# UVA-Computer-Vision-Lab/midvision-probe

Hardware: AMD Instinct MI355X
Metric: images/sec feature-extract+probe-step, ViT-B/16 224^2 (higher is better)
Workload: dtype f16x2 (compensated fp16 pairs of activations and frozen weights, two f16 MFMA products per contraction, fp32 accumulate, feature error as bf16x3; attention: Q.K^T the same two products over compensated pairs, P.V fp16 probabilities x (fp16 + bf16) V; probe, fp32 residual/LN/softmax/loss as in bf16x3

## Files before the change

### midvision-probe_amd/csrc/attention.hip

```cpp
#include "mvp_common.h"

#ifndef MVP_ATT_NT
#define MVP_ATT_NT 0
#endif
#ifndef MVP_ATT_LD_AUX
#define MVP_ATT_LD_AUX 0
#endif
namespace {

#ifndef MVP_ATT_PRIO
#define MVP_ATT_PRIO 0
#endif
#ifndef MVP_ATT_STAGGER
#define MVP_ATT_STAGGER 0
#endif
#if MVP_ATT_PRIO
#define ATT_PRIO(v) __builtin_amdgcn_s_setprio(v)
#else
#define ATT_PRIO(v)
#endif
#ifndef MVP_ATT_ABLATE
#define MVP_ATT_ABLATE 0
#endif
constexpr int TILE = 64 * 128;
constexpr float ATT_DEFER = 6.0f;

template <int SPLIT>
struct AttnState {
  bf16x8_t q_hi[2][2], q_lo[2][2];
  f32x4_t o_acc[4][2];
  float m_run[2], l_run[2];
};

struct AttnBias {
  const float* row[2];
  float scale;
  const float* rel;
  unsigned qoff[2];
  int Kh, Kw, q16, r16;
};

template <int SPLIT, bool LAST, int VF16 = 0, int BIAS = 0>
__device__ __forceinline__ void attn_tile(AttnState<SPLIT>& st, const char* kb, const char* vb, int key0, int N, float cs, int lane,
                                          const AttnBias& ab = AttnBias{}) {
  static_assert(!VF16 || SPLIT == 3, "the fp16-probability form belongs to the bf16x3 mode");
  const int g = lane >> 4, c16 = lane & 15;
  const int nsub = LAST ? min(4, (N - key0 + 15) >> 4) : 4;
  f32x4_t s[4][2];
#pragma unroll
  for (int t = 0; t < 4; ++t)
#pragma unroll
    for (int qt = 0; qt < 2; ++qt) s[t][qt] = f32x4_t{0.f, 0.f, 0.f, 0.f};
  f32x4_t bv[4][2];
  if constexpr (BIAS == 1) {
#pragma unroll
    for (int t = 0; t < 4; ++t)
#pragma unroll
      for (int qt = 0; qt < 2; ++qt)
        bv[t][qt] = (LAST && t >= nsub) ? f32x4_t{0.f, 0.f, 0.f, 0.f} : *(const f32x4_t*)(ab.row[qt] + key0 + t * 16);
  }
  ATT_PRIO(1);
#pragma unroll
  for (int ks = 0; ks < (MVP_ATT_ABLATE == 3 ? 0 : 2); ++ks) {
    const int coff = (((ks << 2) + g) ^ (lane & 7)) << 4;
#pragma unroll
    for (int t = 0; t < 4; ++t) {
      if (LAST && t >= nsub) continue;
      const char* ka = kb + (t * 16 + c16) * 128 + coff;
      const bf16x8_t k_hi = *(const bf16x8_t*)ka;
      if (VF16 == 2) {
        const f16x8_t k_lo = *(const f16x8_t*)(ka + TILE);
        const f16x8_t k_h = __builtin_bit_cast(f16x8_t, k_hi);
#pragma unroll
        for (int qt = 0; qt < 2; ++qt) {
          s[t][qt] = __builtin_amdgcn_mfma_f32_16x16x32_f16(k_lo, __builtin_bit_cast(f16x8_t, st.q_lo[qt][ks]), s[t][qt], 0, 0, 0);
          s[t][qt] = __builtin_amdgcn_mfma_f32_16x16x32_f16(k_h, __builtin_bit_cast(f16x8_t, st.q_hi[qt][ks]), s[t][qt], 0, 0, 0);
        }
        continue;
      }
      if (SPLIT == 3) {
        const bf16x8_t k_lo = *(const bf16x8_t*)(ka + TILE);
#pragma unroll
        for (int qt = 0; qt < 2; ++qt) {
          s[t][qt] = __builtin_amdgcn_mfma_f32_16x16x32_bf16(k_lo, st.q_hi[qt][ks], s[t][qt], 0, 0, 0);
          s[t][qt] = __builtin_amdgcn_mfma_f32_16x16x32_bf16(k_hi, st.q_lo[qt][ks], s[t][qt], 0, 0, 0);
        }
      }
#pragma unroll
      for (int qt = 0; qt < 2; ++qt)
        s[t][qt] = __builtin_amdgcn_mfma_f32_16x16x32_bf16(k_hi, st.q_hi[qt][ks], s[t][qt], 0, 0, 0);
    }
  }
  ATT_PRIO(0);
  if constexpr (BIAS == 1) {
#pragma unroll
    for (int t = 0; t < 4; ++t)
#pragma unroll
      for (int qt = 0; qt < 2; ++qt)
#pragma unroll
        for (int j = 0; j < 4; ++j) s[t][qt][j] = __builtin_fmaf(s[t][qt][j], ab.scale, bv[t][qt][j]);
  }
  if constexpr (BIAS == 2) {
    unsigned k0 = (unsigned)(key0 + g * 4);
    asm volatile("" : "+v"(k0));
    const unsigned Kw4 = (unsigned)ab.Kw << 2, Kh4 = (unsigned)ab.Kh << 2;
    const unsigned q0y = k0 / (unsigned)ab.Kw;
    unsigned ty = q0y << 2, tx = (k0 - q0y * (unsigned)ab.Kw) << 2;
    const char* base = (const char*)ab.rel;
#pragma unroll
    for (int t = 0; t < 4; ++t) {
      if (!(LAST && t >= nsub)) {
        unsigned ky = ty, kx = tx;
#pragma unroll
        for (int j = 0; j < 4; ++j) {
          const bool dead = LAST && (int)k0 + t * 16 + j >= N;
          const unsigned yy = dead ? 0u : ky, xx = (dead ? 0u : kx) + Kh4;
#pragma unroll
          for (int qt = 0; qt < 2; ++qt)
            s[t][qt][j] = __builtin_fmaf(s[t][qt][j], ab.scale, *(const float*)(base + (ab.qoff[qt] + yy)) + *(const float*)(base + (ab.qoff[qt] + xx)));
          kx += 4;
          if (kx == Kw4) {
            kx = 0;
            ky += 4;
          }
        }
      }
      ty += ab.q16;
      tx += ab.r16;
      if (tx >= Kw4) {
        tx -= Kw4;
        ty += 4;
      }
      __builtin_amdgcn_sched_barrier(0);
    }
  }
  const int kbase = key0 + g * 4;
  bf16x8_t p_hi[2][2], p_lo[2][2];
  f16x8_t p_h[2][2];
#pragma unroll
  for (int qt = 0; qt < 2; ++qt) {
    if (VF16 && MVP_ATT_ABLATE != 1) {
      float tmax = -1e30f;
#pragma unroll
      for (int t = 0; t < 4; ++t)
#pragma unroll
        for (int j = 0; j < 4; ++j) {
          if (LAST) s[t][qt][j] = ((kbase + t * 16 + j) < N) ? s[t][qt][j] : -1e30f;
          tmax = fmaxf(tmax, s[t][qt][j]);
        }
      tmax = fmaxf(tmax, __shfl_xor(tmax, 16, 64));
      tmax = fmaxf(tmax, __shfl_xor(tmax, 32, 64));
      if (__builtin_amdgcn_ballot_w64((tmax - st.m_run[qt]) * cs > ATT_DEFER) != 0) {
        const float m_new = fmaxf(st.m_run[qt], tmax);
        const float alpha = __builtin_amdgcn_exp2f((st.m_run[qt] - m_new) * cs);
        st.m_run[qt] = m_new;
        st.l_run[qt] *= alpha;
#pragma unroll
        for (int dt = 0; dt < 4; ++dt) st.o_acc[dt][qt] *= alpha;
      }
      const float mc = st.m_run[qt] * cs;
      float psum = 0.f;
#pragma unroll
      for (int t = 0; t < 4; ++t)
#pragma unroll
        for (int j = 0; j < 4; ++j) {
          const float pv = (LAST && t >= nsub) ? 0.f : __builtin_amdgcn_exp2f(s[t][qt][j] * cs - mc);
          psum += pv;
          p_h[qt][t >> 1][(t & 1) * 4 + j] = (_Float16)pv;
          p_lo[qt][t >> 1][(t & 1) * 4 + j] = (__bf16)pv;
        }
      st.l_run[qt] += psum;
      continue;
    }
    if (MVP_ATT_ABLATE == 1) {
#pragma unroll
      for (int t = 0; t < 4; ++t)
#pragma unroll
        for (int j = 0; j < 4; ++j) {
          p_hi[qt][t >> 1][(t & 1) * 4 + j] = (__bf16)s[t][qt][j];
          if (SPLIT == 3) p_lo[qt][t >> 1][(t & 1) * 4 + j] = (__bf16)(s[t][qt][j] * cs);
        }
      st.l_run[qt] = 1.f;
      continue;
    }
    float tmax = -1e30f;
#pragma unroll
    for (int t = 0; t < 4; ++t)
#pragma unroll
      for (int j = 0; j < 4; ++j) {
        if (LAST) s[t][qt][j] = ((kbase + t * 16 + j) < N) ? s[t][qt][j] : -1e30f;
        tmax = fmaxf(tmax, s[t][qt][j]);
      }
    tmax = fmaxf(tmax, __shfl_xor(tmax, 16, 64));
    tmax = fmaxf(tmax, __shfl_xor(tmax, 32, 64));
    const float m_new = fmaxf(st.m_run[qt], tmax);
    const float alpha = __builtin_amdgcn_exp2f((st.m_run[qt] - m_new) * cs);
    const float mc = m_new * cs;
    st.m_run[qt] = m_new;
    float psum = 0.f;
#pragma unroll
    for (int t = 0; t < 4; ++t)
#pragma unroll
      for (int j = 0; j < 4; ++j) {
        const float pv = (LAST && t >= nsub) ? 0.f : __builtin_amdgcn_exp2f(s[t][qt][j] * cs - mc);
        psum += pv;
        const __bf16 ph = (__bf16)pv;
        p_hi[qt][t >> 1][(t & 1) * 4 + j] = ph;
        if (SPLIT == 3) p_lo[qt][t >> 1][(t & 1) * 4 + j] = (__bf16)(pv - (float)ph);
      }
    st.l_run[qt] = st.l_run[qt] * alpha + psum;
#pragma unroll
    for (int dt = 0; dt < 4; ++dt) st.o_acc[dt][qt] *= alpha;
  }
  const int tr_q = c16 >> 2, tr_p = lane & 3;
  ATT_PRIO(1);
#pragma unroll
  for (int ks = 0; ks < (MVP_ATT_ABLATE == 2 ? 0 : 2); ++ks) {
    if (LAST && 2 * ks >= nsub) continue;
    const int row = ks * 32 + g * 4 + tr_q;
    const int fsw = ((row >> 1) & 3) << 1;
#pragma unroll
    for (int dt = 0; dt < 4; ++dt) {
      const int off = row * 128 + ((((dt << 1) + (tr_p >> 1)) ^ fsw) << 4) + ((tr_p & 1) << 3);
      const bf16x4_t a0 = __builtin_amdgcn_ds_read_tr16_b64_v4bf16((__attribute__((address_space(3))) bf16x4_t*)(vb + off));
      const bf16x4_t a1 = __builtin_amdgcn_ds_read_tr16_b64_v4bf16((__attribute__((address_space(3))) bf16x4_t*)(vb + off + 16 * 128));
      const bf16x8_t v_hi = __builtin_shufflevector(a0, a1, 0, 1, 2, 3, 4, 5, 6, 7);
      if (VF16) {
        const bf16x4_t b0 = __builtin_amdgcn_ds_read_tr16_b64_v4bf16((__attribute__((address_space(3))) bf16x4_t*)(vb + TILE + off));
        const bf16x4_t b1 = __builtin_amdgcn_ds_read_tr16_b64_v4bf16((__attribute__((address_space(3))) bf16x4_t*)(vb + TILE + off + 16 * 128));
        const bf16x8_t v_lo = __builtin_shufflevector(b0, b1, 0, 1, 2, 3, 4, 5, 6, 7);
        const f16x8_t v_h = __builtin_bit_cast(f16x8_t, v_hi);
#pragma unroll
        for (int qt = 0; qt < 2; ++qt) {
          st.o_acc[dt][qt] = __builtin_amdgcn_mfma_f32_16x16x32_bf16(v_lo, p_lo[qt][ks], st.o_acc[dt][qt], 0, 0, 0);
          st.o_acc[dt][qt] = __builtin_amdgcn_mfma_f32_16x16x32_f16(v_h, p_h[qt][ks], st.o_acc[dt][qt], 0, 0, 0);
        }
        continue;
      }
      if (SPLIT == 3) {
        const bf16x4_t b0 = __builtin_amdgcn_ds_read_tr16_b64_v4bf16((__attribute__((address_space(3))) bf16x4_t*)(vb + TILE + off));
        const bf16x4_t b1 = __builtin_amdgcn_ds_read_tr16_b64_v4bf16((__attribute__((address_space(3))) bf16x4_t*)(vb + TILE + off + 16 * 128));
        const bf16x8_t v_lo = __builtin_shufflevector(b0, b1, 0, 1, 2, 3, 4, 5, 6, 7);
#pragma unroll
        for (int qt = 0; qt < 2; ++qt) {
          st.o_acc[dt][qt] = __builtin_amdgcn_mfma_f32_16x16x32_bf16(v_lo, p_hi[qt][ks], st.o_acc[dt][qt], 0, 0, 0);
          st.o_acc[dt][qt] = __builtin_amdgcn_mfma_f32_16x16x32_bf16(v_hi, p_lo[qt][ks], st.o_acc[dt][qt], 0, 0, 0);
        }
      }
#pragma unroll
      for (int qt = 0; qt < 2; ++qt)
        st.o_acc[dt][qt] = __builtin_amdgcn_mfma_f32_16x16x32_bf16(v_hi, p_hi[qt][ks], st.o_acc[dt][qt], 0, 0, 0);
    }
  }
  ATT_PRIO(0);
}

template <int SPLIT>
__device__ __forceinline__ void attn_load_q(AttnState<SPLIT>& st, const mvp_attention_args& p, size_t rowbase, int q0, int h, int lane) {
  const int g = lane >> 4, c16 = lane & 15;
#pragma unroll
  for (int qt = 0; qt < 2; ++qt) {
    const int qrow = min(q0 + qt * 16 + c16, p.N - 1);
    const size_t off = (rowbase + qrow) * p.ld_qkv + h * 64 + g * 8;
#pragma unroll
    for (int ks = 0; ks < 2; ++ks) {
      st.q_hi[qt][ks] = *(const bf16x8_t*)(p.qkv_hi + off + ks * 32);
      if (SPLIT == 3) st.q_lo[qt][ks] = *(const bf16x8_t*)(p.qkv_lo + off + ks * 32);
    }
  }
#pragma unroll
  for (int i = 0; i < 4; ++i)
#pragma unroll
    for (int j = 0; j < 2; ++j) st.o_acc[i][j] = f32x4_t{0.f, 0.f, 0.f, 0.f};
  st.m_run[0] = st.m_run[1] = -1e30f;
  st.l_run[0] = st.l_run[1] = 0.f;
}

template <int SPLIT>
__device__ __forceinline__ void attn_store(AttnState<SPLIT>& st, const mvp_attention_args& p, size_t rowbase, int q0, int h, int lane) {
  const int g = lane >> 4, c16 = lane & 15;
#pragma unroll
  for (int qt = 0; qt < 2; ++qt) {
    float l = st.l_run[qt];
    l += __shfl_xor(l, 16, 64);
    l += __shfl_xor(l, 32, 64);
    const float inv = 1.0f / l;
    const int qrow = q0 + qt * 16 + c16;
    if (qrow >= p.N) continue;
    const bool ilv = p.out_layout == MVP_PAIR_A_ILV32;
    const size_t ob = (rowbase + qrow) * p.ld_out + (ilv ? h * 128 : h * 64) + g * 4;
#pragma unroll
    for (int dt = 0; dt < 4; ++dt) {
      uint32_t h01, l01, h23, l23;
      if (p.out_f16) {
        split2_f16_comp(st.o_acc[dt][qt][0] * inv, st.o_acc[dt][qt][1] * inv, h01, l01);
        split2_f16_comp(st.o_acc[dt][qt][2] * inv, st.o_acc[dt][qt][3] * inv, h23, l23);
      } else {
        split2_bf16(st.o_acc[dt][qt][0] * inv, st.o_acc[dt][qt][1] * inv, h01, l01);
        split2_bf16(st.o_acc[dt][qt][2] * inv, st.o_acc[dt][qt][3] * inv, h23, l23);
      }
      if (ilv) {
        const size_t o = ob + (dt >> 1) * 64 + (dt & 1) * 16;
        store_out((u32x2_t*)(p.out_hi + o), u32x2_t{h01, h23}, MVP_ATT_NT);
        store_out((u32x2_t*)(p.out_hi + o + 32), u32x2_t{l01, l23}, MVP_ATT_NT);
      } else {
        store_out((u32x2_t*)(p.out_hi + ob + dt * 16), u32x2_t{h01, h23}, MVP_ATT_NT);
        if (p.out_lo) store_out((u32x2_t*)(p.out_lo + ob + dt * 16), u32x2_t{l01, l23}, MVP_ATT_NT);
      }
    }
  }
}

template <int SPLIT>
__device__ __forceinline__ void attn_stage_piece(const mvp_attention_args& p, size_t rowbase, int h, int key0, int r, char* kdst, char* vdst, int lane) {
  const int rsub = lane >> 3;
  const int kc = ((lane & 7) ^ rsub) << 3;
  const int vc = ((lane & 7) ^ (((lane >> 4) & 3) << 1)) << 3;
  const int HD = p.H * 64;
  if (MVP_ATT_ABLATE == 4) return;
  const int krow = min(key0 + r + rsub, p.N - 1);
  const size_t ro = (rowbase + krow) * p.ld_qkv + h * 64;
  __builtin_amdgcn_global_load_lds(GLB_PTR(p.qkv_hi + ro + HD + kc), LDS_PTR(kdst + r * 128), 16, 0, MVP_ATT_LD_AUX);
  __builtin_amdgcn_global_load_lds(GLB_PTR(p.qkv_hi + ro + 2 * HD + vc), LDS_PTR(vdst + r * 128), 16, 0, MVP_ATT_LD_AUX);
  if (SPLIT == 3) {
    __builtin_amdgcn_global_load_lds(GLB_PTR(p.qkv_lo + ro + HD + kc), LDS_PTR(kdst + TILE + r * 128), 16, 0, MVP_ATT_LD_AUX);
    __builtin_amdgcn_global_load_lds(GLB_PTR(p.qkv_lo + ro + 2 * HD + vc), LDS_PTR(vdst + TILE + r * 128), 16, 0, MVP_ATT_LD_AUX);
  }
}

template <int BIAS> struct AttnKArgs { typedef mvp_attention_args type; };
template <> struct AttnKArgs<1> { typedef mvp_attention_bias_args type; };
template <> struct AttnKArgs<2> { typedef mvp_attention_relpos_args type; };
__host__ __device__ __forceinline__ const mvp_attention_args& att_of(const mvp_attention_args& a) { return a; }
__host__ __device__ __forceinline__ const mvp_attention_args& att_of(const mvp_attention_bias_args& a) { return a.att; }
__host__ __device__ __forceinline__ const mvp_attention_args& att_of(const mvp_attention_relpos_args& a) { return a.att; }
__device__ __forceinline__ void attn_bias_rows(AttnBias& ab, const mvp_attention_bias_args& a, int bh, int h, int q0, int lane) {
  const int g = lane >> 4, c16 = lane & 15;
#pragma unroll
  for (int qt = 0; qt < 2; ++qt)
    ab.row[qt] = a.bias + (size_t)h * (size_t)a.bias_head_stride + (size_t)min(q0 + qt * 16 + c16, a.att.N - 1) * (size_t)a.ld_bias + g * 4;
}
__device__ __forceinline__ void attn_bias_rows(AttnBias& ab, const mvp_attention_relpos_args& a, int bh, int h, int q0, int lane) {
  const int c16 = lane & 15;
#pragma unroll
  for (int qt = 0; qt < 2; ++qt) ab.qoff[qt] = ((unsigned)min(q0 + qt * 16 + c16, a.att.N - 1) * (unsigned)a.ld_rel) << 2;
}
__device__ __forceinline__ void attn_bias_rows(AttnBias&, const mvp_attention_args&, int, int, int, int) {}
__device__ __forceinline__ void attn_bias_pair(AttnBias& ab, const mvp_attention_relpos_args& a, int bh) { ab.rel = a.rel + (size_t)bh * (size_t)a.rel_bh_stride; }
__device__ __forceinline__ void attn_bias_pair(AttnBias&, const mvp_attention_bias_args&, int) {}
__device__ __forceinline__ void attn_bias_pair(AttnBias&, const mvp_attention_args&, int) {}
__device__ __forceinline__ void attn_bias_init(AttnBias& ab, const mvp_attention_relpos_args& a) {
  ab.Kh = a.Kh;
  ab.Kw = a.Kw;
  ab.q16 = (16 / a.Kw) << 2;
  ab.r16 = (16 % a.Kw) << 2;
}
__device__ __forceinline__ void attn_bias_init(AttnBias&, const mvp_attention_bias_args&) {}
__device__ __forceinline__ void attn_bias_init(AttnBias&, const mvp_attention_args&) {}

template <int SPLIT, int VF16 = 0, int BIAS = 0>
__global__ __launch_bounds__(256) void attention_stream_kernel(const typename AttnKArgs<BIAS>::type pa) {
  const mvp_attention_args& p = att_of(pa);
  f16_saturate_mode();
  extern __shared__ __attribute__((aligned(16))) char smem[];
  constexpr int NARR = (SPLIT == 3) ? 2 : 1;
  constexpr int STAGE = 2 * NARR * TILE;
  const int lane = threadIdx.x & 63, wave = threadIdx.x >> 6;
  const int bh = blockIdx.y, b = bh / p.H, h = bh - b * p.H;
  const int q0 = blockIdx.x * 128 + wave * 32;
  const int nkt = (p.N + 63) >> 6;
  const size_t rowbase = (size_t)b * p.N;
  AttnState<SPLIT> st;
  attn_load_q<SPLIT>(st, p, rowbase, q0, h, lane);
  const float cs = BIAS ? 1.44269504088896340736f : p.scale * 1.44269504088896340736f;
  const bool active = q0 < p.N;
  AttnBias ab{};
  if constexpr (BIAS != 0) {
    ab.scale = p.scale;
    attn_bias_init(ab, pa);
    attn_bias_pair(ab, pa, bh);
    if (active) attn_bias_rows(ab, pa, bh, h, q0, lane);
  }

  auto stage = [&](int buf, int kt) {
    char* base = smem + buf * STAGE;
#pragma unroll
    for (int ps = 0; ps < 2; ++ps) attn_stage_piece<SPLIT>(p, rowbase, h, kt * 64, ps * 32 + wave * 8, base, base + NARR * TILE, lane);
  };
  stage(0, 0);
  asm volatile("s_waitcnt vmcnt(0)" ::: "memory");
  __syncthreads();
  for (int kt = 0; kt < nkt; ++kt) {
    if (kt + 1 < nkt) stage((kt + 1) & 1, kt + 1);
    if (active) {
      const char* kb = smem + (kt & 1) * STAGE;
      if (kt == nkt - 1) attn_tile<SPLIT, true, VF16, BIAS>(st, kb, kb + NARR * TILE, kt * 64, p.N, cs, lane, ab);
      else attn_tile<SPLIT, false, VF16, BIAS>(st, kb, kb + NARR * TILE, kt * 64, p.N, cs, lane, ab);
    }
    asm volatile("s_waitcnt vmcnt(0)" ::: "memory");
    __syncthreads();
  }
  if (active) attn_store<SPLIT>(st, p, rowbase, q0, h, lane);
}

template <int SPLIT, int VF16 = 0, int BIAS = 0>
__global__ __launch_bounds__(512) void attention_resident_kernel(const typename AttnKArgs<BIAS>::type pa) {
  const mvp_attention_args& p = att_of(pa);
  f16_saturate_mode();
  extern __shared__ __attribute__((aligned(16))) char smem[];
  constexpr int NARR = (SPLIT == 3) ? 2 : 1;
  constexpr int STAGE = 2 * NARR * TILE;
  const int lane = threadIdx.x & 63, wave = threadIdx.x >> 6;
  const int q0 = wave * 32;
  const int nkt = (p.N + 63) >> 6, nslot = nkt + 1;
  const int npair = p.B * p.H;
  const float cs = BIAS ? 1.44269504088896340736f : p.scale * 1.44269504088896340736f;
  const bool active = q0 < p.N;
  const int g = lane >> 4, c16 = lane & 15;
  AttnBias ab{};
  if constexpr (BIAS != 0) {
    ab.scale = p.scale;
    attn_bias_init(ab, pa);
  }

  auto stage_tile = [&](int bh, int kt, int slot) {
    const int b = bh / p.H, h = bh - b * p.H;
    char* base = smem + slot * STAGE;
    attn_stage_piece<SPLIT>(p, (size_t)b * p.N, h, kt * 64, wave * 8, base, base + NARR * TILE, lane);
  };
  bf16x8_t qn_hi[2][2], qn_lo[2][2];
  auto fetch_q = [&](int bh) {
    const int b = bh / p.H, h = bh - b * p.H;
#pragma unroll
    for (int qt = 0; qt < 2; ++qt) {
      const int qrow = min(q0 + qt * 16 + c16, p.N - 1);
      const size_t off = ((size_t)b * p.N + qrow) * p.ld_qkv + h * 64 + g * 8;
#pragma unroll
      for (int ks = 0; ks < 2; ++ks) {
        qn_hi[qt][ks] = *(const bf16x8_t*)(p.qkv_hi + off + ks * 32);
        if (SPLIT == 3) qn_lo[qt][ks] = *(const bf16x8_t*)(p.qkv_lo + off + ks * 32);
      }
    }
  };

  int bh = blockIdx.x;
  if (bh >= npair) return;
  stage_tile(bh, 0, 0);
  fetch_q(bh);
  asm volatile("s_waitcnt vmcnt(0)" ::: "memory");
  __syncthreads();
  AttnState<SPLIT> st;
  for (int i = 0; bh < npair; ++i, bh += gridDim.x) {
    const int b = bh / p.H, h = bh - b * p.H;
    const size_t rowbase = (size_t)b * p.N;
    const int s0 = (nkt * i) % nslot;
    if constexpr (BIAS != 0) {
      attn_bias_pair(ab, pa, bh);
      if (active) attn_bias_rows(ab, pa, bh, h, q0, lane);
    }
    for (int kt = 1; kt < nkt; ++kt) stage_tile(bh, kt, (s0 + kt) % nslot);
#pragma unroll
    for (int qt = 0; qt < 2; ++qt)
#pragma unroll
      for (int ks = 0; ks < 2; ++ks) {
        st.q_hi[qt][ks] = qn_hi[qt][ks];
        if (SPLIT == 3) st.q_lo[qt][ks] = qn_lo[qt][ks];
      }
#pragma unroll
    for (int a = 0; a < 4; ++a)
#pragma unroll
      for (int c = 0; c < 2; ++c) st.o_acc[a][c] = f32x4_t{0.f, 0.f, 0.f, 0.f};
    st.m_run[0] = st.m_run[1] = -1e30f;
    st.l_run[0] = st.l_run[1] = 0.f;
    if (active && MVP_ATT_ABLATE != 5) {
      const char* kb = smem + s0 * STAGE;
      if (nkt == 1) attn_tile<SPLIT, true, VF16, BIAS>(st, kb, kb + NARR * TILE, 0, p.N, cs, lane, ab);
      else attn_tile<SPLIT, false, VF16, BIAS>(st, kb, kb + NARR * TILE, 0, p.N, cs, lane, ab);
    }
    asm volatile("s_waitcnt vmcnt(0)" ::: "memory");
    __syncthreads();
    if (MVP_ATT_STAGGER && wave >= 4) __builtin_amdgcn_s_sleep(MVP_ATT_STAGGER);
    const int nbh = bh + gridDim.x;
    if (nbh < npair) {
      stage_tile(nbh, 0, (s0 + nkt) % nslot);
      fetch_q(nbh);
    }
    if (active) {
      for (int kt = 1; kt < (MVP_ATT_ABLATE == 5 ? 0 : nkt); ++kt) {
        const char* kb = smem + ((s0 + kt) % nslot) * STAGE;
        if (kt == nkt - 1) attn_tile<SPLIT, true, VF16, BIAS>(st, kb, kb + NARR * TILE, kt * 64, p.N, cs, lane, ab);
        else attn_tile<SPLIT, false, VF16, BIAS>(st, kb, kb + NARR * TILE, kt * 64, p.N, cs, lane, ab);
      }
    }
    asm volatile("s_waitcnt vmcnt(0)" ::: "memory");
    if (active) attn_store<SPLIT>(st, p, rowbase, q0, h, lane);
    if (nbh < npair) __builtin_amdgcn_s_barrier();
    if (MVP_ATT_STAGGER && wave >= 4) __builtin_amdgcn_s_sleep(MVP_ATT_STAGGER);
  }
}

template <int SPLIT, int VF16 = 0, int BIAS = 0>
int launch_attention(const typename AttnKArgs<BIAS>::type* ka, hipStream_t s) {
  const mvp_attention_args* a = &att_of(*ka);
  constexpr int NARR = (SPLIT == 3) ? 2 : 1;
  constexpr int STAGE = 2 * NARR * TILE;
  constexpr int SMEM_STREAM = 2 * STAGE, SMEM_RES = 5 * STAGE;
  static int configured = [] {
    int e = (int)hipFuncSetAttribute((const void*)attention_stream_kernel<SPLIT, VF16, BIAS>, hipFuncAttributeMaxDynamicSharedMemorySize, SMEM_STREAM);
    if (e == 0) e = (int)hipFuncSetAttribute((const void*)attention_resident_kernel<SPLIT, VF16, BIAS>, hipFuncAttributeMaxDynamicSharedMemorySize, SMEM_RES);
    return e;
  }();
  if (configured != 0) return MVP_ELAUNCH;
  if (a->N <= 256) {
    const int nkt = (a->N + 63) >> 6;
    static const int cus = [] {
      int dev = 0, n = 0;
      if (hipGetDevice(&dev) != hipSuccess || hipDeviceGetAttribute(&n, hipDeviceAttributeMultiprocessorCount, dev) != hipSuccess) n = 0;
      return n > 0 ? n : 256;
    }();
    const int per_cu = (160 * 1024) / ((nkt + 1) * STAGE) > 0 ? (160 * 1024) / ((nkt + 1) * STAGE) : 1;
    const int grid = a->B * a->H < cus * per_cu ? a->B * a->H : cus * per_cu;
    hipLaunchKernelGGL((attention_resident_kernel<SPLIT, VF16, BIAS>), dim3(grid), dim3(512), (nkt + 1) * STAGE, s, *ka);
  } else {
    dim3 grid((a->N + 127) / 128, a->B * a->H);
    hipLaunchKernelGGL((attention_stream_kernel<SPLIT, VF16, BIAS>), grid, dim3(256), SMEM_STREAM, s, *ka);
  }
  MVP_LAUNCH_CHECK();
  return MVP_OK;
}

}

static int attention_check(const mvp_attention_args* a) {
  if (!a || !a->qkv_hi || !a->out_hi) return MVP_EINVAL;
  if (a->B <= 0 || a->N <= 0 || a->H <= 0) return MVP_EINVAL;
  if ((a->ld_qkv & 7) || (a->ld_out & 3) || a->ld_qkv < 3 * a->H * 64 || a->ld_out < a->H * 64) return MVP_EINVAL;
  if (a->out_layout != MVP_PAIR_SEPARATE && (a->out_layout != MVP_PAIR_A_ILV32 || a->precision != MVP_PREC_BF16X3 || a->ld_out < 2 * a->H * 64)) return MVP_EINVAL;
  if (a->precision == MVP_PREC_BF16X3) {
    if (!a->qkv_lo || (!a->out_lo && a->out_layout == MVP_PAIR_SEPARATE)) return MVP_EINVAL;
    if (a->v_format != MVP_ATT_V_F16 && a->v_format != MVP_ATT_V_F16_QK_F16 && a->v_format != MVP_ATT_V_BF16_PAIR) return MVP_EINVAL;
    return MVP_OK;
  }
  if (a->precision != MVP_PREC_BF16 || a->v_format != MVP_ATT_V_BF16_PAIR || a->out_f16) return MVP_EINVAL;
  return MVP_OK;
}

template <int BIAS>
static int attention_dispatch(const typename AttnKArgs<BIAS>::type* ka, hipStream_t s) {
  const mvp_attention_args* a = &att_of(*ka);
  if (a->precision == MVP_PREC_BF16X3) {
    if (a->v_format == MVP_ATT_V_F16) return launch_attention<3, 1, BIAS>(ka, s);
    if (a->v_format == MVP_ATT_V_F16_QK_F16) return launch_attention<3, 2, BIAS>(ka, s);
    return launch_attention<3, 0, BIAS>(ka, s);
  }
  return launch_attention<1, 0, BIAS>(ka, s);
}

extern "C" int mvp_attention_fwd(const mvp_attention_args* a, void* stream) {
  if (attention_check(a) != MVP_OK) return MVP_EINVAL;
  return attention_dispatch<0>(a, (hipStream_t)stream);
}

extern "C" int mvp_attention_bias_fwd(const mvp_attention_bias_args* a, void* stream) {
  if (!a || attention_check(&a->att) != MVP_OK) return MVP_EINVAL;
  if (!a->bias || ((uintptr_t)a->bias & 15)) return MVP_EINVAL;
  const int64_t npad = 64 * (((int64_t)a->att.N + 63) / 64);
  if ((a->ld_bias & 3) || a->ld_bias < npad) return MVP_EINVAL;
  if (a->bias_head_stride < (int64_t)a->att.N * a->ld_bias || (a->bias_head_stride & 3)) return MVP_EINVAL;
  return attention_dispatch<1>(a, (hipStream_t)stream);
}

extern "C" int mvp_attention_relpos_fwd(const mvp_attention_relpos_args* a, void* stream) {
  if (!a || attention_check(&a->att) != MVP_OK) return MVP_EINVAL;
  if (!a->rel || ((uintptr_t)a->rel & 3)) return MVP_EINVAL;
  if (a->Kh <= 0 || a->Kw <= 0 || (int64_t)a->Kh * a->Kw != (int64_t)a->att.N) return MVP_EINVAL;
  if ((int64_t)a->ld_rel < (int64_t)a->Kh + a->Kw || a->rel_bh_stride < (int64_t)a->att.N * a->ld_rel) return MVP_EINVAL;
  if ((int64_t)a->att.N * a->ld_rel >= (1ll << 30)) return MVP_EINVAL;
  return attention_dispatch<2>(a, (hipStream_t)stream);
}
```

### midvision-probe_amd/csrc/tokens.hip

```cpp
#include "mvp_common.h"

namespace {

__global__ __launch_bounds__(256) void split_kernel(const mvp_split_bf16_args p) {
  const int64_t n4 = p.n >> 2;
  for (int64_t i = (int64_t)blockIdx.x * 256 + threadIdx.x; i < n4; i += (int64_t)gridDim.x * 256) {
    const float4 v = ((const float4*)p.src)[i];
    uint16_t h[4], l[4];
    split_bf16(v.x, h[0], l[0]); split_bf16(v.y, h[1], l[1]);
    split_bf16(v.z, h[2], l[2]); split_bf16(v.w, h[3], l[3]);
    ((u32x2_t*)p.hi)[i] = u32x2_t{pack2(h[0], h[1]), pack2(h[2], h[3])};
    if (p.lo) ((u32x2_t*)p.lo)[i] = u32x2_t{pack2(l[0], l[1]), pack2(l[2], l[3])};
  }
  if (blockIdx.x == 0 && threadIdx.x < (p.n & 3)) {
    const int64_t i = (n4 << 2) + threadIdx.x;
    uint16_t h, l;
    split_bf16(p.src[i], h, l);
    p.hi[i] = h;
    if (p.lo) p.lo[i] = l;
  }
}

__global__ __launch_bounds__(256) void patch_gather_kernel(const mvp_patch_gather_args p) {
  const int P = p.P, PP = P * P, Kc = p.C * PP;
  const int64_t rows = (int64_t)p.B * p.gh * p.gw;
  const int64_t total4 = rows * (Kc >> 2);
  const bool vec = ((p.W & 3) == 0) && ((p.pad_left & 3) == 0);
  for (int64_t i = (int64_t)blockIdx.x * 256 + threadIdx.x; i < total4; i += (int64_t)gridDim.x * 256) {
    const int64_t row = i / (Kc >> 2);
    const int col = (int)(i - row * (Kc >> 2)) << 2;
    const int c = col / PP, rem = col - c * PP, ky = rem / P, kx = rem - ky * P;
    const int b = (int)(row / (p.gh * p.gw));
    const int pr = (int)(row - (int64_t)b * p.gh * p.gw);
    const int py = pr / p.gw, px = pr - py * p.gw;
    const int y = py * P + ky - p.pad_top;
    const int x = px * P + kx - p.pad_left;
    float v[4] = {0.f, 0.f, 0.f, 0.f};
    if (y >= 0 && y < p.H) {
      const float* src = p.images + (((size_t)b * p.C + c) * p.H + y) * p.W;
      if (vec && x >= 0 && x + 3 < p.W) {
        const float4 t = *(const float4*)(src + x);
        v[0] = t.x; v[1] = t.y; v[2] = t.z; v[3] = t.w;
      } else {
#pragma unroll
        for (int e = 0; e < 4; ++e)
          if (x + e >= 0 && x + e < p.W) v[e] = src[x + e];
      }
    }
    uint16_t h[4], l[4];
#pragma unroll
    for (int e = 0; e < 4; ++e) split_bf16(v[e], h[e], l[e]);
    const size_t o = (size_t)row * Kc + col;
    *(u32x2_t*)(p.out_hi + o) = u32x2_t{pack2(h[0], h[1]), pack2(h[2], h[3])};
    if (p.out_lo) *(u32x2_t*)(p.out_lo + o) = u32x2_t{pack2(l[0], l[1]), pack2(l[2], l[3])};
  }
}

__global__ __launch_bounds__(256) void patch_gather_ld_kernel(const mvp_patch_gather_ld_args pa) {
  const mvp_patch_gather_args& p = pa.g;
  const int P = p.P, PP = P * P, Kc = p.C * PP, ld4 = pa.ldk >> 2;
  const int64_t rows = (int64_t)p.B * p.gh * p.gw;
  const int64_t total4 = rows * ld4;
  for (int64_t i = (int64_t)blockIdx.x * 256 + threadIdx.x; i < total4; i += (int64_t)gridDim.x * 256) {
    const int64_t row = i / ld4;
    const int col = (int)(i - row * ld4) << 2;
    const int b = (int)(row / (p.gh * p.gw));
    const int pr = (int)(row - (int64_t)b * p.gh * p.gw);
    const int py = pr / p.gw, px = pr - py * p.gw;
    float v[4] = {0.f, 0.f, 0.f, 0.f};
    if (col < Kc) {
#pragma unroll
      for (int e = 0; e < 4; ++e) {
        const int k = col + e;
        const int c = k / PP, rem = k - c * PP, ky = rem / P, kx = rem - ky * P;
        const int y = py * P + ky - p.pad_top, x = px * P + kx - p.pad_left;
        if (y >= 0 && y < p.H && x >= 0 && x < p.W) v[e] = p.images[(((size_t)b * p.C + c) * p.H + y) * p.W + x];
      }
    }
    uint16_t h[4], l[4];
#pragma unroll
    for (int e = 0; e < 4; ++e) split_bf16(v[e], h[e], l[e]);
    const size_t o = (size_t)row * pa.ldk + col;
    *(u32x2_t*)(p.out_hi + o) = u32x2_t{pack2(h[0], h[1]), pack2(h[2], h[3])};
    if (p.out_lo) *(u32x2_t*)(p.out_lo + o) = u32x2_t{pack2(l[0], l[1]), pack2(l[2], l[3])};
  }
}

__global__ __launch_bounds__(256) void cls_rows_kernel(const mvp_cls_rows_args p) {
  const int i = blockIdx.x * 256 + threadIdx.x;
  if (i >= p.B * p.C) return;
  const int b = i / p.C, c = i - b * p.C;
  p.x[(size_t)b * p.N * p.C + c] = p.cls[c] + p.pos0[c];
}

__global__ __launch_bounds__(256) void prefix_rows_kernel(const mvp_prefix_rows_args p) {
  const int64_t i = (int64_t)blockIdx.x * 256 + threadIdx.x;
  const int per = (1 + p.R) * p.C;
  if (i >= (int64_t)p.B * per) return;
  const int b = (int)(i / per), j = (int)(i - (int64_t)b * per);
  const int r = j / p.C, c = j - r * p.C;
  p.x[((size_t)b * p.N + r) * p.C + c] = r == 0 ? p.cls[c] + p.pos0[c] : p.reg[(size_t)(r - 1) * p.C + c];
}

constexpr int BN_RB = 8;

__host__ __device__ inline int bn_slab_rows(int M) {
  int rb = BN_RB;
  while ((M + rb - 1) / rb > 2048) rb <<= 1;
  return rb;
}

__global__ __launch_bounds__(256) void bn_partial_kernel(const float* __restrict__ x, float* __restrict__ part, int M, int C, int rb) {
  x += (size_t)blockIdx.z * M * C;
  part += (size_t)blockIdx.z * gridDim.x * C * 3;
  const int r0 = blockIdx.x * rb;
  const int nr = min(rb, M - r0);
  const int c = blockIdx.y * 256 + threadIdx.x;
  if (c >= C) return;
  const float* col = x + (size_t)r0 * C + c;
  const float shift = col[0];
  float s1 = 0.f, s2 = 0.f;
  for (int rr = 0; rr < nr; rr += BN_RB) {
    float v[BN_RB];
#pragma unroll
    for (int r = 0; r < BN_RB; ++r) v[r] = col[(size_t)min(rr + r, nr - 1) * C];
#pragma unroll
    for (int r = 0; r < BN_RB; ++r) {
      const float d = (rr + r < nr) ? v[r] - shift : 0.f;
      s1 += d;
      s2 += d * d;
    }
  }
  float* o = part + ((size_t)blockIdx.x * C + c) * 3;
  o[0] = shift; o[1] = s1; o[2] = s2;
}

constexpr int BN_FC = 16, BN_FG = 64;

__device__ __forceinline__ float bn_running(float old, float val, float momentum) {
#pragma clang fp contract(off)
  const float a = (1.f - momentum) * old;
  const float b = momentum * val;
  return a + b;
}

__global__ __launch_bounds__(1024) void bn_finalize_kernel(mvp_bn_tokens_args p, const float* __restrict__ part,
                                                           float* __restrict__ ss, int M, int nslab, int rb) {
  __shared__ double red[BN_FG][BN_FC][2];
  part += (size_t)blockIdx.y * nslab * p.C * 3;
  ss += (size_t)blockIdx.y * 2 * p.C;
  p.stats += (size_t)blockIdx.y * p.stats_gstride;
  const int lc = threadIdx.x & (BN_FC - 1), grp = threadIdx.x / BN_FC;
  const int c = blockIdx.x * BN_FC + lc;
  const bool ok = c < p.C;
  const double ref = ok ? (double)part[(size_t)c * 3] : 0.0;
  double s1 = 0.0, s2 = 0.0;
  if (ok) {
    for (int s0 = grp; s0 < nslab; s0 += BN_FG * 4) {
      float o0[4], o1[4], o2[4];
#pragma unroll
      for (int u = 0; u < 4; ++u) {
        const int s = min(s0 + u * BN_FG, nslab - 1);
        const float* o = part + ((size_t)s * p.C + c) * 3;
        o0[u] = o[0]; o1[u] = o[1]; o2[u] = o[2];
      }
#pragma unroll
      for (int u = 0; u < 4; ++u) {
        const int s = s0 + u * BN_FG;
        if (s < nslab) {
          const double nb = (double)min(rb, M - s * rb);
          const double d = (double)o0[u] - ref, a1 = (double)o1[u], a2 = (double)o2[u];
          s1 += a1 + nb * d;
          s2 += a2 + 2.0 * d * a1 + nb * d * d;
        }
      }
    }
  }
  red[grp][lc][0] = s1;
  red[grp][lc][1] = s2;
  __syncthreads();
  if (grp != 0 || !ok) return;
  s1 = 0.0; s2 = 0.0;
#pragma unroll 8
  for (int g = 0; g < BN_FG; ++g) { s1 += red[g][lc][0]; s2 += red[g][lc][1]; }
  const double n = (double)M;
  const double dm = s1 / n;
  const double mean = ref + dm;
  const double m2 = fmax(s2 - s1 * dm, 0.0);
  const double var = m2 / n;
  p.stats[c] = (float)mean;
  p.stats[p.C + c] = (float)var;
  const double unb = (n > 1.0) ? m2 / (n - 1.0) : var;
  if (p.defer_running) {
    p.stats[2 * p.C + c] = (float)unb;
  } else if (p.running_mean) {
    p.running_mean[c] = bn_running(p.running_mean[c], (float)mean, p.momentum);
    p.running_var[c] = bn_running(p.running_var[c], (float)unb, p.momentum);
  }
  const float rstd = rsqrtf((float)var + p.eps);
  const float g = p.gamma ? p.gamma[c] : 1.f, b = p.beta ? p.beta[c] : 0.f;
  ss[c] = rstd * g;
  ss[p.C + c] = b - (float)mean * rstd * g;
  if (c == 0 && p.num_batches_tracked && !p.defer_running) *p.num_batches_tracked += 1;
}

__global__ __launch_bounds__(256) void bn_running_update_kernel(const mvp_bn_running_update_args p) {
  const int c = blockIdx.x * 256 + threadIdx.x;
  if (c == 0 && p.num_batches_tracked) *p.num_batches_tracked += 1;
  if (c >= p.C) return;
  p.running_mean[c] = bn_running(p.running_mean[c], p.stats[c], p.momentum);
  p.running_var[c] = bn_running(p.running_var[c], p.stats[2 * p.C + c], p.momentum);
}

struct bn_running_update_set { mvp_bn_running_update_args item[MVP_BN_RUNNING_MAX]; };
__global__ __launch_bounds__(256) void bn_running_update_n_kernel(const bn_running_update_set s) {
  const mvp_bn_running_update_args& p = s.item[blockIdx.y];
  const int c = blockIdx.x * 256 + threadIdx.x;
  if (c == 0 && p.num_batches_tracked) *p.num_batches_tracked += 1;
  if (c >= p.C) return;
  p.running_mean[c] = bn_running(p.running_mean[c], p.stats[c], p.momentum);
  p.running_var[c] = bn_running(p.running_var[c], p.stats[2 * p.C + c], p.momentum);
}

__global__ __launch_bounds__(256) void bn_prep_kernel(const mvp_bn_tokens_args p, float* __restrict__ ss) {
  const int c = blockIdx.x * 256 + threadIdx.x;
  if (c >= p.C) return;
  ss += (size_t)blockIdx.y * 2 * p.C;
  if (p.mode == 2) {
    ss[c] = 1.f; ss[p.C + c] = 0.f;
    return;
  }
  const float rstd = rsqrtf(p.running_var[c] + p.eps);
  const float g = p.gamma ? p.gamma[c] : 1.f, b = p.beta ? p.beta[c] : 0.f;
  ss[c] = rstd * g;
  ss[p.C + c] = b - p.running_mean[c] * rstd * g;
}

__global__ __launch_bounds__(256) void bn_apply_kernel(mvp_bn_tokens_args p, const float* __restrict__ ss) {
  __shared__ float tile[32][65];
  if (blockIdx.z) {
    const size_t g = blockIdx.z;
    p.x += g * p.B * p.N * p.C;
    ss += g * 2 * p.C;
    if (p.nchw) p.nchw += g * p.nchw_gstride;
    if (p.tok_hi) p.tok_hi += g * p.tok_gstride;
    if (p.tok_lo) p.tok_lo += g * p.tok_gstride;
    if (p.cls_out) p.cls_out += g * p.cls_gstride;
  }
  const int t = threadIdx.x;
  const int ptiles = (p.hw + 31) / 32;
  const int b = blockIdx.x / ptiles, pt = blockIdx.x - b * ptiles;
  const int p0 = pt * 32, c0 = blockIdx.y * 64;
  const int tok0 = p.N - p.hw;
  {
    const int c = c0 + (t & 63);
    const float sc = (c < p.C) ? ss[c] : 0.f, sh = (c < p.C) ? ss[p.C + c] : 0.f;
    if (p.cls_out && pt == 0 && t < 64 && c < p.C) p.cls_out[(size_t)b * p.C + c] = p.x[(size_t)b * p.N * p.C + c] * sc + sh;
#pragma unroll
    for (int i = 0; i < 8; ++i) {
      const int tp = i * 4 + (t >> 6), pp = p0 + tp;
      float y = 0.f;
      if (pp < p.hw && c < p.C) {
        y = p.x[((size_t)b * p.N + tok0 + pp) * p.C + c] * sc + sh;
        if (p.tok_hi) {
          uint16_t h, l;
          split_bf16(y, h, l);
          const size_t o = ((size_t)b * p.hw + pp) * p.ld_tok + p.col_off + c;
          p.tok_hi[o] = h;
          if (p.tok_lo) p.tok_lo[o] = l;
        }
      }
      tile[tp][t & 63] = y;
    }
  }
  __syncthreads();
#pragma unroll
  for (int i = 0; i < 8; ++i) {
    const int cc = i * 8 + (t >> 5), tp = t & 31;
    const int c = c0 + cc, pp = p0 + tp;
    if (c < p.C && pp < p.hw) {
      const float y = tile[tp][cc];
      if (p.nchw) p.nchw[((size_t)b * p.C + c) * p.hw + pp] = y;
      if (p.tokT_hi) {
        uint16_t h, l;
        split_bf16(y, h, l);
        const size_t o = (size_t)(p.col_off + c) * p.ldT + (size_t)b * p.hw + pp;
        p.tokT_hi[o] = h;
        if (p.tokT_lo) p.tokT_lo[o] = l;
      }
    }
  }
}

__global__ __launch_bounds__(256) void pack_nchw_kernel(const mvp_pack_nchw_args p) {
  __shared__ float tile[64][33];
  const int t = threadIdx.x;
  const int ptiles = (p.hw + 31) / 32;
  const int b = blockIdx.x / ptiles, pt = blockIdx.x - b * ptiles;
  const int p0 = pt * 32, c0 = blockIdx.y * 64;
#pragma unroll
  for (int i = 0; i < 8; ++i) {
    const int cc = i * 8 + (t >> 5), tp = t & 31;
    const int c = c0 + cc, pp = p0 + tp;
    float y = 0.f;
    if (c < p.C && pp < p.hw) {
      y = p.nchw[((size_t)b * p.C + c) * p.hw + pp];
      if (p.tokT_hi) {
        uint16_t h, l;
        split_bf16(y, h, l);
        const size_t o = (size_t)(p.col_off + c) * p.ldT + (size_t)b * p.hw + pp;
        p.tokT_hi[o] = h;
        if (p.tokT_lo) p.tokT_lo[o] = l;
      }
    }
    tile[cc][tp] = y;
  }
  __syncthreads();
  if (!p.tok_hi) return;
#pragma unroll
  for (int i = 0; i < 8; ++i) {
    const int tp = i * 4 + (t >> 6), cc = t & 63;
    const int c = c0 + cc, pp = p0 + tp;
    if (c < p.C && pp < p.hw) {
      uint16_t h, l;
      split_bf16(tile[cc][tp], h, l);
      const size_t o = ((size_t)b * p.hw + pp) * p.ld_tok + p.col_off + c;
      p.tok_hi[o] = h;
      if (p.tok_lo) p.tok_lo[o] = l;
    }
  }
}

inline int grid_for(int64_t work, int cap = 2048) {
  int64_t g = (work + 255) / 256;
  if (g < 1) g = 1;
  if (g > cap) g = cap;
  return (int)g;
}

}

extern "C" int mvp_split_bf16(const mvp_split_bf16_args* a, void* stream) {
  if (!a || !a->src || !a->hi || a->n <= 0) return MVP_EINVAL;
  hipLaunchKernelGGL(split_kernel, dim3(grid_for(a->n >> 2)), dim3(256), 0, (hipStream_t)stream, *a);
  MVP_LAUNCH_CHECK();
  return MVP_OK;
}

extern "C" int mvp_patch_gather(const mvp_patch_gather_args* a, void* stream) {
  if (!a || !a->images || !a->out_hi) return MVP_EINVAL;
  if (a->P <= 0 || (a->P & 3) || a->B <= 0 || a->C <= 0) return MVP_EINVAL;
  if (a->gh * a->P < a->H + a->pad_top || a->gw * a->P < a->W + a->pad_left) return MVP_EINVAL;
  const int64_t total4 = (int64_t)a->B * a->gh * a->gw * ((a->C * a->P * a->P) >> 2);
  hipLaunchKernelGGL(patch_gather_kernel, dim3(grid_for(total4, 4096)), dim3(256), 0, (hipStream_t)stream, *a);
  MVP_LAUNCH_CHECK();
  return MVP_OK;
}

extern "C" int mvp_patch_gather_ld(const mvp_patch_gather_ld_args* a, void* stream) {
  if (!a || !a->g.images || !a->g.out_hi) return MVP_EINVAL;
  const mvp_patch_gather_args& g = a->g;
  if (g.P <= 0 || g.B <= 0 || g.C <= 0 || g.gh <= 0 || g.gw <= 0 || g.pad_top < 0 || g.pad_left < 0) return MVP_EINVAL;
  if (((g.C * g.P * g.P) & 3) || (a->ldk & 3) || a->ldk < g.C * g.P * g.P) return MVP_EINVAL;
  if (g.gh * g.P < g.H + g.pad_top || g.gw * g.P < g.W + g.pad_left) return MVP_EINVAL;
  if (((size_t)g.out_hi & 7) || ((size_t)g.out_lo & 7)) return MVP_EINVAL;
  const int64_t total4 = (int64_t)g.B * g.gh * g.gw * (a->ldk >> 2);
  hipLaunchKernelGGL(patch_gather_ld_kernel, dim3(grid_for(total4, 4096)), dim3(256), 0, (hipStream_t)stream, *a);
  MVP_LAUNCH_CHECK();
  return MVP_OK;
}

extern "C" int mvp_prefix_rows(const mvp_prefix_rows_args* a, void* stream) {
  if (!a || !a->cls || !a->pos0 || !a->x || a->B <= 0 || a->C <= 0 || a->R < 0 || a->N < 1 + a->R || (a->R > 0 && !a->reg)) return MVP_EINVAL;
  const int64_t n = (int64_t)a->B * (1 + a->R) * a->C;
  hipLaunchKernelGGL(prefix_rows_kernel, dim3((unsigned)((n + 255) / 256)), dim3(256), 0, (hipStream_t)stream, *a);
  MVP_LAUNCH_CHECK();
  return MVP_OK;
}

extern "C" int mvp_cls_rows(const mvp_cls_rows_args* a, void* stream) {
  if (!a || !a->cls || !a->pos0 || !a->x || a->B <= 0 || a->C <= 0) return MVP_EINVAL;
  hipLaunchKernelGGL(cls_rows_kernel, dim3((a->B * a->C + 255) / 256), dim3(256), 0, (hipStream_t)stream, *a);
  MVP_LAUNCH_CHECK();
  return MVP_OK;
}

extern "C" int64_t mvp_bn_tokens_workspace_bytes(int M, int C) {
  const int rb = bn_slab_rows(M);
  const int64_t nslab = (M + rb - 1) / rb;
  return (nslab * C * 3 + 2 * (int64_t)C) * 4;
}

extern "C" int mvp_bn_tokens_to_nchw_fwd(const mvp_bn_tokens_args* a, void* stream) {
  if (!a || !a->x || !a->workspace) return MVP_EINVAL;
  if (a->B <= 0 || a->N <= 0 || a->C <= 0 || a->hw <= 0 || a->hw > a->N) return MVP_EINVAL;
  const int M = a->B * a->N;
  const int G = a->groups > 1 ? a->groups : 1;
  if (a->workspace_bytes < G * mvp_bn_tokens_workspace_bytes(M, a->C)) return MVP_EINVAL;
  if (a->mode == 0 && !a->stats) return MVP_EINVAL;
  if (a->defer_running && a->mode != 0) return MVP_EINVAL;
  if (a->mode == 1 && (!a->running_mean || !a->running_var)) return MVP_EINVAL;
  if (G > 1) {
    if ((a->mode == 0 && !a->defer_running) || a->tokT_hi || G > 65535) return MVP_EINVAL;
    if (a->stats_gstride < 0 || a->nchw_gstride < 0 || a->tok_gstride < 0 || a->cls_gstride < 0) return MVP_EINVAL;
  }
  hipStream_t s = (hipStream_t)stream;
  const int rb = bn_slab_rows(M);
  const int nslab = (M + rb - 1) / rb;
  float* part = (float*)a->workspace;
  float* ss = part + (size_t)G * nslab * a->C * 3;
  if (a->mode == 0) {
    hipLaunchKernelGGL(bn_partial_kernel, dim3(nslab, (a->C + 255) / 256, G), dim3(256), 0, s, a->x, part, M, a->C, rb);
    hipLaunchKernelGGL(bn_finalize_kernel, dim3((a->C + BN_FC - 1) / BN_FC, G), dim3(1024), 0, s, *a, part, ss, M, nslab, rb);
  } else {
    hipLaunchKernelGGL(bn_prep_kernel, dim3((a->C + 255) / 256, G), dim3(256), 0, s, *a, ss);
  }
  if (a->cls_out && a->N <= a->hw) return MVP_EINVAL;
  if (a->nchw || a->tok_hi || a->tokT_hi || a->cls_out) {
    const int ptiles = (a->hw + 31) / 32;
    hipLaunchKernelGGL(bn_apply_kernel, dim3(a->B * ptiles, (a->C + 63) / 64, G), dim3(256), 0, s, *a, ss);
  }
  MVP_LAUNCH_CHECK();
  return MVP_OK;
}

extern "C" int mvp_bn_running_update(const mvp_bn_running_update_args* a, void* stream) {
  if (!a || !a->stats || !a->running_mean || !a->running_var || a->C <= 0) return MVP_EINVAL;
  hipLaunchKernelGGL(bn_running_update_kernel, dim3((a->C + 255) / 256), dim3(256), 0, (hipStream_t)stream, *a);
  MVP_LAUNCH_CHECK();
  return MVP_OK;
}

extern "C" int mvp_bn_running_update_n(const mvp_bn_running_update_args* items, int n, void* stream) {
  if (!items || n <= 0 || n > MVP_BN_RUNNING_MAX) return MVP_EINVAL;
  bn_running_update_set s;
  int cmax = 0;
  for (int i = 0; i < n; ++i) {
    const mvp_bn_running_update_args& a = items[i];
    if (!a.stats || !a.running_mean || !a.running_var || a.C <= 0) return MVP_EINVAL;
    for (int j = 0; j < i; ++j)
      if (items[j].running_mean == a.running_mean || items[j].running_var == a.running_var) return MVP_EINVAL;
    s.item[i] = a;
    cmax = a.C > cmax ? a.C : cmax;
  }
  for (int i = n; i < MVP_BN_RUNNING_MAX; ++i) s.item[i] = items[0];
  hipLaunchKernelGGL(bn_running_update_n_kernel, dim3((cmax + 255) / 256, n), dim3(256), 0, (hipStream_t)stream, s);
  MVP_LAUNCH_CHECK();
  return MVP_OK;
}

extern "C" int mvp_pack_nchw_tokens(const mvp_pack_nchw_args* a, void* stream) {
  if (!a || !a->nchw || (!a->tok_hi && !a->tokT_hi)) return MVP_EINVAL;
  if (a->B <= 0 || a->C <= 0 || a->hw <= 0) return MVP_EINVAL;
  const int ptiles = (a->hw + 31) / 32;
  hipLaunchKernelGGL(pack_nchw_kernel, dim3(a->B * ptiles, (a->C + 63) / 64), dim3(256), 0, (hipStream_t)stream, *a);
  MVP_LAUNCH_CHECK();
  return MVP_OK;
}

namespace {
__global__ __launch_bounds__(256) void gather_rows_kernel(const mvp_gather_rows_args p, const unsigned chunks, const unsigned total) {
  const unsigned i = blockIdx.x * 256u + threadIdx.x;
  if (i >= total) return;
  const unsigned r = i / chunks, c = (i - r * chunks) << 3;
  const int s = p.idx[r];
  const bool live = s >= 0 && s < p.rows_in;
  const size_t so = (size_t)(live ? s : 0) * p.ld_in + c, o = (size_t)r * p.ld_out + c;
  const u32x4_t z = {0u, 0u, 0u, 0u};
  *(u32x4_t*)(p.out_hi + o) = live ? *(const u32x4_t*)(p.in_hi + so) : z;
  if (p.out_lo) *(u32x4_t*)(p.out_lo + o) = live ? *(const u32x4_t*)(p.in_lo + so) : z;
}
}

extern "C" int mvp_gather_rows(const mvp_gather_rows_args* a, void* stream) {
  if (!a || !a->in_hi || !a->out_hi || !a->idx) return MVP_EINVAL;
  if ((a->in_lo == nullptr) != (a->out_lo == nullptr)) return MVP_EINVAL;
  if (a->rows <= 0 || a->rows_in <= 0 || a->cols <= 0 || (a->cols & 7)) return MVP_EINVAL;
  if (a->ld_in < a->cols || a->ld_out < a->cols || (a->ld_in & 7) || (a->ld_out & 7)) return MVP_EINVAL;
  if (((size_t)a->in_hi & 15) || ((size_t)a->in_lo & 15) || ((size_t)a->out_hi & 15) || ((size_t)a->out_lo & 15) || ((size_t)a->idx & 3)) return MVP_EINVAL;
  const int64_t chunks = a->cols >> 3, total = (int64_t)a->rows * chunks;
  if (total > 0x7fffffffll) return MVP_EINVAL;
  hipLaunchKernelGGL(gather_rows_kernel, dim3((unsigned)((total + 255) / 256)), dim3(256), 0, (hipStream_t)stream, *a, (unsigned)chunks, (unsigned)total);
  MVP_LAUNCH_CHECK();
  return MVP_OK;
}
```

Before: 11380.

## Split tail attention pairs across half-blocks and add vectorized BN apply kernel

The resident attention kernel now divides the final partial wave of (batch, head) pairs so that two blocks share one tail pair, each handling half the query rows by wave group. This is meant to reduce the tail imbalance when the pair count does not divide the grid. A separate BN apply kernel processes 224 tokens per block with 8-wide vector loads and stores, then transposes through shared memory for the NCHW output. It is used when alignment allows and is meant to cut memory transaction count. Env knobs for grid cap and the tail split are also added.

Measured after the change: 11450, median of 6. Within noise of the previous version (+0.6%).

```diff
diff --git a/midvision-probe_amd/csrc/attention.hip b/midvision-probe_amd/csrc/attention.hip
--- a/midvision-probe_amd/csrc/attention.hip
+++ b/midvision-probe_amd/csrc/attention.hip
@@ -404,7 +404,7 @@
 }
 
 template <int SPLIT, int VF16 = 0, int BIAS = 0>
-__global__ __launch_bounds__(512) void attention_resident_kernel(const typename AttnKArgs<BIAS>::type pa) {
+__global__ __launch_bounds__(512) void attention_resident_kernel(const typename AttnKArgs<BIAS>::type pa, const int tail_split) {
   const mvp_attention_args& p = att_of(pa);
   f16_saturate_mode();
   extern __shared__ __attribute__((aligned(16))) char smem[];
@@ -415,13 +415,18 @@
   const int nkt = (p.N + 63) >> 6, nslot = nkt + 1;
   const int npair = p.B * p.H;
   const float cs = BIAS ? 1.44269504088896340736f : p.scale * 1.44269504088896340736f;
-  const bool active = q0 < p.N;
+  const bool has_rows = q0 < p.N;
   const int g = lane >> 4, c16 = lane & 15;
   AttnBias ab{};
   if constexpr (BIAS != 0) {
     ab.scale = p.scale;
     attn_bias_init(ab, pa);
   }
+  const int G = gridDim.x, w = blockIdx.x;
+  const int R = npair / G, rem = npair - R * G;
+  const bool split = tail_split && rem > 0 && 2 * rem <= G && p.N > 128;
+  const int tail_bh = R * G + (split ? w >> 1 : w);
+  const int nit = R + ((split ? w < 2 * rem : w < rem) ? 1 : 0);
 
   auto stage_tile = [&](int bh, int kt, int slot) {
     const int b = bh / p.H, h = bh - b * p.H;
@@ -443,14 +448,15 @@
     }
   };
 
-  int bh = blockIdx.x;
-  if (bh >= npair) return;
+  if (nit == 0) return;
+  int bh = R > 0 ? w : tail_bh;
   stage_tile(bh, 0, 0);
   fetch_q(bh);
   asm volatile("s_waitcnt vmcnt(0)" ::: "memory");
   __syncthreads();
   AttnState<SPLIT> st;
-  for (int i = 0; bh < npair; ++i, bh += gridDim.x) {
+  for (int i = 0; i < nit; ++i) {
+    const bool active = has_rows && (!(split && i == R) || (wave >> 2) == (w & 1));
     const int b = bh / p.H, h = bh - b * p.H;
     const size_t rowbase = (size_t)b * p.N;
     const int s0 = (nkt * i) % nslot;
@@ -480,8 +486,9 @@
     asm volatile("s_waitcnt vmcnt(0)" ::: "memory");
     __syncthreads();
     if (MVP_ATT_STAGGER && wave >= 4) __builtin_amdgcn_s_sleep(MVP_ATT_STAGGER);
-    const int nbh = bh + gridDim.x;
-    if (nbh < npair) {
+    const bool more = i + 1 < nit;
+    const int nbh = i + 1 < R ? bh + G : tail_bh;
+    if (more) {
       stage_tile(nbh, 0, (s0 + nkt) % nslot);
       fetch_q(nbh);
     }
@@ -494,8 +501,9 @@
     }
     asm volatile("s_waitcnt vmcnt(0)" ::: "memory");
     if (active) attn_store<SPLIT>(st, p, rowbase, q0, h, lane);
-    if (nbh < npair) __builtin_amdgcn_s_barrier();
+    if (more) __builtin_amdgcn_s_barrier();
     if (MVP_ATT_STAGGER && wave >= 4) __builtin_amdgcn_s_sleep(MVP_ATT_STAGGER);
+    bh = nbh;
   }
 }
 
@@ -519,8 +527,13 @@
       return n > 0 ? n : 256;
     }();
     const int per_cu = (160 * 1024) / ((nkt + 1) * STAGE) > 0 ? (160 * 1024) / ((nkt + 1) * STAGE) : 1;
-    const int grid = a->B * a->H < cus * per_cu ? a->B * a->H : cus * per_cu;
-    hipLaunchKernelGGL((attention_resident_kernel<SPLIT, VF16, BIAS>), dim3(grid), dim3(512), (nkt + 1) * STAGE, s, *ka);
+    int grid = a->B * a->H < cus * per_cu ? a->B * a->H : cus * per_cu;
+    const char* eg = getenv("MVP_ATT_GRID");
+    const int cap = eg ? atoi(eg) : 0;
+    if (cap > 0 && cap < grid) grid = cap;
+    const char* es = getenv("MVP_ATT_TAIL_SPLIT");
+    const int tail_split = es ? (atoi(es) != 0) : 1;
+    hipLaunchKernelGGL((attention_resident_kernel<SPLIT, VF16, BIAS>), dim3(grid), dim3(512), (nkt + 1) * STAGE, s, *ka, tail_split);
   } else {
     dim3 grid((a->N + 127) / 128, a->B * a->H);
     hipLaunchKernelGGL((attention_stream_kernel<SPLIT, VF16, BIAS>), grid, dim3(256), SMEM_STREAM, s, *ka);
diff --git a/midvision-probe_amd/csrc/tokens.hip b/midvision-probe_amd/csrc/tokens.hip
--- a/midvision-probe_amd/csrc/tokens.hip
+++ b/midvision-probe_amd/csrc/tokens.hip
@@ -292,6 +292,97 @@
   }
 }
 
+constexpr int BN_AT = 224;
+constexpr int BN_AP = BN_AT + 1;
+__global__ __launch_bounds__(256) void bn_apply8_kernel(mvp_bn_tokens_args p, const float* __restrict__ ss) {
+  __shared__ float tile[64 * BN_AP];
+  if (blockIdx.z) {
+    const size_t g = blockIdx.z;
+    p.x += g * p.B * p.N * p.C;
+    ss += g * 2 * p.C;
+    if (p.nchw) p.nchw += g * p.nchw_gstride;
+    if (p.tok_hi) p.tok_hi += g * p.tok_gstride;
+    if (p.tok_lo) p.tok_lo += g * p.tok_gstride;
+    if (p.cls_out) p.cls_out += g * p.cls_gstride;
+  }
+  const int t = threadIdx.x;
+  const int nchunk = (p.hw + BN_AT - 1) / BN_AT;
+  const int b = blockIdx.x / nchunk, pt = blockIdx.x - b * nchunk;
+  const int p0 = pt * BN_AT, c0 = blockIdx.y * 64;
+  const int nt = min(BN_AT, p.hw - p0);
+  const int tok0 = p.N - p.hw;
+  {
+    const int cl = (t & 7) * 8, c = c0 + cl;
+    const bool cok = c < p.C;
+    f32x4_t sc[2], sh[2];
+#pragma unroll
+    for (int u = 0; u < 2; ++u) {
+      sc[u] = cok ? *(const f32x4_t*)(ss + c + 4 * u) : f32x4_t{0.f, 0.f, 0.f, 0.f};
+      sh[u] = cok ? *(const f32x4_t*)(ss + p.C + c + 4 * u) : f32x4_t{0.f, 0.f, 0.f, 0.f};
+    }
+    if (p.cls_out && pt == 0 && t < 8 && cok) {
+      const float* xr = p.x + (size_t)b * p.N * p.C + c;
+#pragma unroll
+      for (int u = 0; u < 2; ++u) {
+        const f32x4_t xv = *(const f32x4_t*)(xr + 4 * u);
+#pragma unroll
+        for (int k = 0; k < 4; ++k) p.cls_out[(size_t)b * p.C + c + 4 * u + k] = xv[k] * sc[u][k] + sh[u][k];
+      }
+    }
+    f32x4_t xv[BN_AT / 32][2];
+#pragma unroll
+    for (int i = 0; i < BN_AT / 32; ++i) {
+      const int tp = i * 32 + (t >> 3);
+      if (tp < nt && cok) {
+        const float* xr = p.x + ((size_t)b * p.N + tok0 + p0 + tp) * p.C + c;
+        xv[i][0] = *(const f32x4_t*)xr;
+        xv[i][1] = *(const f32x4_t*)(xr + 4);
+      }
+    }
+#pragma unroll
+    for (int i = 0; i < BN_AT / 32; ++i) {
+      const int tp = i * 32 + (t >> 3);
+      if (tp < nt && cok) {
+        float y[8];
+#pragma unroll
+        for (int u = 0; u < 2; ++u)
+#pragma unroll
+          for (int k = 0; k < 4; ++k) y[4 * u + k] = xv[i][u][k] * sc[u][k] + sh[u][k];
+        if (p.tok_hi) {
+          u32x4_t h, l;
+#pragma unroll
+          for (int k = 0; k < 4; ++k) {
+            uint32_t hh, ll;
+            split2_bf16(y[2 * k], y[2 * k + 1], hh, ll);
+            h[k] = hh;
+            l[k] = ll;
+          }
+          const size_t o = ((size_t)b * p.hw + p0 + tp) * p.ld_tok + p.col_off + c;
+          *(u32x4_t*)(p.tok_hi + o) = h;
+          if (p.tok_lo) *(u32x4_t*)(p.tok_lo + o) = l;
+        }
+#pragma unroll
+        for (int k = 0; k < 8; ++k) tile[(cl + k) * BN_AP + tp] = y[k];
+      }
+    }
+  }
+  if (!p.nchw) return;
+  __syncthreads();
+  const int dq = 256 / nt, dr = 256 - dq * nt;
+  int cc = t / nt, pp = t - cc * nt;
+  float* out = p.nchw + ((size_t)b * p.C + c0) * p.hw + p0;
+  const int ncc = min(64, p.C - c0);
+  while (cc < ncc) {
+    out[(size_t)cc * p.hw + pp] = tile[cc * BN_AP + pp];
+    cc += dq;
+    pp += dr;
+    if (pp >= nt) {
+      pp -= nt;
+      ++cc;
+    }
+  }
+}
+
 __global__ __launch_bounds__(256) void pack_nchw_kernel(const mvp_pack_nchw_args p) {
   __shared__ float tile[64][33];
   const int t = threadIdx.x;
@@ -417,8 +508,15 @@
   }
   if (a->cls_out && a->N <= a->hw) return MVP_EINVAL;
   if (a->nchw || a->tok_hi || a->tokT_hi || a->cls_out) {
-    const int ptiles = (a->hw + 31) / 32;
-    hipLaunchKernelGGL(bn_apply_kernel, dim3(a->B * ptiles, (a->C + 63) / 64, G), dim3(256), 0, s, *a, ss);
+    const bool x16 = !(((uintptr_t)a->x | (uintptr_t)a->workspace) & 15);
+    const bool tok16 = !a->tok_hi || (!(((uintptr_t)a->tok_hi | (uintptr_t)a->tok_lo) & 15) && !(a->ld_tok & 7) && !(a->col_off & 7) && (G == 1 || !(a->tok_gstride & 7)));
+    if (x16 && !(a->C & 7) && !a->tokT_hi && tok16) {
+      const int ptiles = (a->hw + BN_AT - 1) / BN_AT;
+      hipLaunchKernelGGL(bn_apply8_kernel, dim3(a->B * ptiles, (a->C + 63) / 64, G), dim3(256), 0, s, *a, ss);
+    } else {
+      const int ptiles = (a->hw + 31) / 32;
+      hipLaunchKernelGGL(bn_apply_kernel, dim3(a->B * ptiles, (a->C + 63) / 64, G), dim3(256), 0, s, *a, ss);
+    }
   }
   MVP_LAUNCH_CHECK();
   return MVP_OK;
```
